# Hello1024/shared-tensor

Measured on AMD Instinct MI355X. Metric: async-DP tokens/sec GPT-2-small, higher is better.
Workload: dtype bf16; 1 GPU; model=gpt2-small, global_batch=64, seq_len=1024, parallelism=async-dp1, codec=1bit, n_params=124439808, paramsync=n/a at n_gpus=1 (no links)

## Files before the change

build.py:

```python
#!/usr/bin/env python3
import argparse
import hashlib
import os
import subprocess
import sysconfig

ROOT = os.path.dirname(os.path.abspath(__file__))
CSRC = os.path.join(ROOT, "sharedtensor_amd", "csrc")
OUT = os.path.join(ROOT, "sharedtensor_amd", "_core.so")
BUILD = os.path.join(ROOT, "build")

SOURCES = [
    "codec_cpu.cpp",
    "engine.cpp",
    "rccl_transport.cpp",
    "hip_kernels.hip",
    "ln_kernels.hip",
    "ce_kernels.hip",
    "gelu_kernels.hip",
    "swiglu_kernels.hip",
    "bindings.cpp",
]

HEADERS = ["common.h", "codec_cpu.h", "engine.h", "hip_api.h", "rccl_transport.h"]


def pybind11_include():
    import pybind11
    return pybind11.get_include()


def build(force=False, debug=False, verbose=True):
    os.makedirs(BUILD, exist_ok=True)
    py_inc = sysconfig.get_paths()["include"]
    rocm = os.environ.get("ROCM_PATH", "/opt/rocm")
    hipcc = os.path.join(rocm, "bin", "hipcc")
    cxxflags = [
        "--offload-arch=gfx950",
        "-std=c++20",
        "-O3" if not debug else "-O0",
        "-g" if debug else "",
        "-fPIC",
        "-DSHAMD_WITH_HIP",
        f"-I{CSRC}",
        f"-I{py_inc}",
        f"-I{pybind11_include()}",
        f"-I{rocm}/include",
        "-Wno-unused-result",
        "-fvisibility=hidden",
        "-DNDEBUG" if not debug else "",
        "-parallel-jobs=4",
    ]
    cxxflags = [f for f in cxxflags if f]

    h = hashlib.sha256()
    for f in SOURCES + HEADERS:
        with open(os.path.join(CSRC, f), "rb") as fh:
            h.update(fh.read())
    h.update(" ".join(cxxflags).encode())
    stamp = os.path.join(BUILD, "core.stamp")
    digest = h.hexdigest()
    if not force and os.path.exists(OUT) and os.path.exists(stamp):
        with open(stamp) as fh:
            if fh.read().strip() == digest:
                if verbose:
                    print(f"[build.py] {OUT} up to date")
                return OUT

    objs = []
    procs = []
    for src in SOURCES:
        obj = os.path.join(BUILD, src.replace("/", "_") + ".o")
        objs.append(obj)
        cmd = [hipcc, "-c", os.path.join(CSRC, src), "-o", obj] + cxxflags
        if verbose:
            print("[build.py]", " ".join(cmd))
        procs.append(subprocess.Popen(cmd))
    rc = 0
    for p in procs:
        rc |= p.wait()
    if rc:
        raise RuntimeError("hipcc compilation failed")

    link = [hipcc, "-shared", "-fPIC", "-o", OUT] + objs + [
        f"-L{rocm}/lib", "-lamdhip64", "-lrccl", "-pthread",
        f"-Wl,-rpath,{rocm}/lib",
    ]
    if verbose:
        print("[build.py]", " ".join(link))
    subprocess.check_call(link)
    nm = subprocess.run(["nm", "-C", "-u", OUT], capture_output=True, text=True)
    bad = [l for l in nm.stdout.splitlines() if "shamd::" in l]
    if bad:
        raise RuntimeError("unresolved engine symbols:\n" + "\n".join(bad))
    with open(stamp, "w") as fh:
        fh.write(digest)
    if verbose:
        print(f"[build.py] built {OUT}")
    return OUT


if __name__ == "__main__":
    ap = argparse.ArgumentParser()
    ap.add_argument("--force", action="store_true")
    ap.add_argument("--debug", action="store_true")
    args = ap.parse_args()
    build(force=args.force, debug=args.debug)
```

sharedtensor_amd/csrc/bindings.cpp:

```cpp
#include <pybind11/pybind11.h>
#include <pybind11/stl.h>

#include "codec_cpu.h"
#include "engine.h"
#include "rccl_transport.h"

namespace py = pybind11;
using namespace shamd;

namespace {

py::tuple py_cpu_encode(int codec, uintptr_t delta, int64_t n, double scale_in,
                        uintptr_t payload_out) {
  Codec c = static_cast<Codec>(codec);
  float* d = reinterpret_cast<float*>(delta);
  float scale = scale_in < 0 ? cpu_compute_scale(c, d, n)
                             : static_cast<float>(scale_in);
  cpu_quantize(c, d, n, scale, reinterpret_cast<uint8_t*>(payload_out));
  return py::make_tuple(scale, payload_bytes(c, n));
}

void py_cpu_apply(int codec, uintptr_t payload, int64_t n, double scale,
                  std::vector<uintptr_t> dsts) {
  std::vector<float*> d;
// ... 138 lines not shown
      .def("copy_to", &Engine::copy_to,
           py::call_guard<py::gil_scoped_release>())
      .def("fused_sgd", &Engine::fused_sgd,
           py::call_guard<py::gil_scoped_release>())
      .def("fused_sgd_bf16", &Engine::fused_sgd_bf16,
           py::call_guard<py::gil_scoped_release>())
      .def("fused_adamw", &Engine::fused_adamw,
           py::call_guard<py::gil_scoped_release>())
      .def("notify_dirty", &Engine::notify_dirty)
      .def("close", &Engine::close, py::call_guard<py::gil_scoped_release>())
      .def("is_master", &Engine::is_master)
      .def("listen_port", &Engine::listen_port)
      .def("last_error", &Engine::last_error)
      .def("reconnect_count", &Engine::reconnect_count)
      .def("recent_scales_sent", &Engine::recent_scales_sent)
      .def("recent_scales_recv", &Engine::recent_scales_recv)
      .def("link_stats", [](Engine& e) {
        py::list out;
        for (auto& s : e.link_stats()) {
          py::dict d;
          d["rounds_sent"] = s.rounds_sent;
          d["rounds_recv"] = s.rounds_recv;
          d["bytes_sent"] = s.bytes_sent;
          d["bytes_recv"] = s.bytes_recv;
          d["last_scale_sent"] = s.last_scale_sent;
          d["last_scale_recv"] = s.last_scale_recv;
          d["active"] = s.active;
          d["dead"] = s.dead;
          d["peer"] = s.peer;
          d["rccl"] = s.rccl;
          out.append(d);
        }
        return out;
      });

  py::class_<DevCodec>(m, "DevCodec")
      .def(py::init<int, std::vector<int64_t>, int, bool>(), py::arg("codec"),
           py::arg("sizes"), py::arg("device"), py::arg("delta_bf16") = false)
      .def("reduce_scales", &DevCodec::reduce_scales)
      .def("quantize", &DevCodec::quantize, py::arg("delta"),
           py::arg("scales"), py::arg("payload"), py::arg("stream"),
           py::arg("stats") = 0)
      .def("finalize_scales", &DevCodec::finalize_scales)
      .def("apply", &DevCodec::apply);
  m.def("gpu_add_scatter", &py_gpu_add_scatter, py::arg("src"), py::arg("n"),
        py::arg("alpha"), py::arg("dsts"), py::arg("stream"),
        py::arg("delta_bf16") = false);
  m.def("gpu_fused_sgd", &py_gpu_fused_sgd, py::arg("mom"), py::arg("grad"),
        py::arg("lr"), py::arg("mu"), py::arg("n"), py::arg("dsts"),
        py::arg("stream"), py::arg("delta_bf16") = false);
  m.def("rccl_loopback_payload", &rccl_loopback_payload,
        "Self ncclSend/ncclRecv of a real payload on one device (1-rank "
        "comm): executes the non-blocking enqueue ordering + stream polling "
        "the 2-GPU xGMI links use and verifies the moved bytes.");
  m.def("rccl_self_test", &rccl_self_test,
        py::call_guard<py::gil_scoped_release>());

  m.def("gelu_fwd", [](uintptr_t x, uintptr_t y, int64_t n, uintptr_t stream) {
    hip_gelu_fwd(reinterpret_cast<const void*>(x), reinterpret_cast<void*>(y),
                 n, reinterpret_cast<hipStream_t>(stream));
  });
  m.def("gelu_bwd", [](uintptr_t dy, uintptr_t x, uintptr_t dx, int64_t n,
                       uintptr_t stream) {
    hip_gelu_bwd(reinterpret_cast<const void*>(dy),
                 reinterpret_cast<const void*>(x),
                 reinterpret_cast<void*>(dx), n,
                 reinterpret_cast<hipStream_t>(stream));
  });

  m.def("ce_fwd", [](uintptr_t logits, uintptr_t targets, uintptr_t loss,
                     uintptr_t row_m, uintptr_t row_lse, int64_t R, int64_t V,
                     uintptr_t stream) {
    hip_ce_fwd(reinterpret_cast<const void*>(logits),
               reinterpret_cast<const int32_t*>(targets),
               reinterpret_cast<float*>(loss), reinterpret_cast<float*>(row_m),
               reinterpret_cast<float*>(row_lse), R, V,
               reinterpret_cast<hipStream_t>(stream));
  });
  m.def("ce_bwd", [](uintptr_t logits, uintptr_t targets, uintptr_t row_lse,
                     uintptr_t dlogits, uintptr_t gscale_dev, double inv_r,
                     int64_t R, int64_t V, uintptr_t stream) {
    hip_ce_bwd(reinterpret_cast<const void*>(logits),
               reinterpret_cast<const int32_t*>(targets),
               reinterpret_cast<const float*>(row_lse),
               reinterpret_cast<void*>(dlogits),
               reinterpret_cast<const float*>(gscale_dev),
               static_cast<float>(inv_r), R, V,
               reinterpret_cast<hipStream_t>(stream));
  });

  m.def("ln_fwd", [](uintptr_t x, uintptr_t w, uintptr_t b, uintptr_t y,
                     uintptr_t mean, uintptr_t rstd, int64_t R, int C,
                     double eps, uintptr_t stream) {
    hip_ln_fwd(reinterpret_cast<const void*>(x),
               reinterpret_cast<const void*>(w),
               reinterpret_cast<const void*>(b), reinterpret_cast<void*>(y),
               reinterpret_cast<float*>(mean), reinterpret_cast<float*>(rstd),
               R, C, static_cast<float>(eps),
               reinterpret_cast<hipStream_t>(stream));
  });
  m.def("colsum_bf16", [](uintptr_t x, uintptr_t out, int64_t R, int C,
                          uintptr_t stream) {
    hip_colsum_bf16(reinterpret_cast<const void*>(x),
                    reinterpret_cast<float*>(out), R, C,
                    reinterpret_cast<hipStream_t>(stream));
  });
  m.def("swiglu_fwd", [](uintptr_t x1, uintptr_t x3, uintptr_t y, int64_t n,
                         uintptr_t stream) {
    hip_swiglu_fwd(reinterpret_cast<const void*>(x1),
                   reinterpret_cast<const void*>(x3),
                   reinterpret_cast<void*>(y), n,
                   reinterpret_cast<hipStream_t>(stream));
  });
  m.def("swiglu_bwd", [](uintptr_t dy, uintptr_t x1, uintptr_t x3,
                         uintptr_t dx1, uintptr_t dx3, int64_t n,
                         uintptr_t stream) {
    hip_swiglu_bwd(reinterpret_cast<const void*>(dy),
                   reinterpret_cast<const void*>(x1),
                   reinterpret_cast<const void*>(x3),
                   reinterpret_cast<void*>(dx1),
                   reinterpret_cast<void*>(dx3), n,
                   reinterpret_cast<hipStream_t>(stream));
  });
  m.def("rms_fwd", [](uintptr_t x, uintptr_t w, uintptr_t y, uintptr_t rstd,
                      int64_t R, int C, double eps, uintptr_t stream) {
    hip_rms_fwd(reinterpret_cast<const void*>(x),
                reinterpret_cast<const void*>(w), reinterpret_cast<void*>(y),
                reinterpret_cast<float*>(rstd), R, C, static_cast<float>(eps),
                reinterpret_cast<hipStream_t>(stream));
  });
  m.def("rms_bwd", [](uintptr_t dy, uintptr_t x, uintptr_t w, uintptr_t rstd,
                      uintptr_t dx, uintptr_t dgamma, int64_t R, int C,
                      uintptr_t stream) {
    hip_rms_bwd(reinterpret_cast<const void*>(dy),
                reinterpret_cast<const void*>(x),
                reinterpret_cast<const void*>(w),
                reinterpret_cast<const float*>(rstd),
                reinterpret_cast<void*>(dx), reinterpret_cast<float*>(dgamma),
                R, C, reinterpret_cast<hipStream_t>(stream));
  });
  m.def("ln_bwd", [](uintptr_t dy, uintptr_t x, uintptr_t w, uintptr_t mean,
                     uintptr_t rstd, uintptr_t dx, uintptr_t dgamma,
                     uintptr_t dbeta, int64_t R, int C, uintptr_t stream) {
    hip_ln_bwd(reinterpret_cast<const void*>(dy),
               reinterpret_cast<const void*>(x),
               reinterpret_cast<const void*>(w),
               reinterpret_cast<const float*>(mean),
               reinterpret_cast<const float*>(rstd),
               reinterpret_cast<void*>(dx), reinterpret_cast<float*>(dgamma),
               reinterpret_cast<float*>(dbeta), R, C,
               reinterpret_cast<hipStream_t>(stream));
  });

  m.def("msg_bytes", &Engine::msg_bytes);
  m.def("scales_area", &Engine::scales_area);
  m.def("payload_bytes",
        [](int c, int64_t n) { return payload_bytes(static_cast<Codec>(c), n); });
  m.def("pad64", &pad64);
  m.def("cpu_encode", &py_cpu_encode);
  m.def("cpu_apply", &py_cpu_apply);
  m.def("cpu_scale", &py_cpu_scale);
  m.def("f32_to_e4m3", [](float x) { return static_cast<int>(f32_to_e4m3(x)); });
  m.def("e4m3_to_f32", [](int v) { return e4m3_to_f32(static_cast<uint8_t>(v)); });

#ifdef SHAMD_WITH_HIP
  m.attr("with_hip") = true;
#else
  m.attr("with_hip") = false;
#endif
}
```

sharedtensor_amd/csrc/codec_cpu.cpp:

```cpp
#include "codec_cpu.h"

#include <atomic>
#include <cmath>
#include <cstdlib>
#include <cstring>
#include <thread>
#include <vector>

namespace shamd {

static constexpr int64_t PF_CHUNK = int64_t(1) << 22;

static int cpu_codec_threads() {
  static const int t = [] {
    const char* e = std::getenv("SHTENS_CPU_THREADS");
    if (e) {
      int v = std::atoi(e);
      return v < 1 ? 1 : v;
    }
    unsigned hw = std::thread::hardware_concurrency();
    return static_cast<int>(hw < 1 ? 1 : (hw > 16 ? 16 : hw));
  }();
  return t;
}

void cpu_pfor(int64_t n, const std::function<void(int64_t, int64_t)>& fn) {
  if (n <= 0) return;
  int64_t nchunks = (n + PF_CHUNK - 1) / PF_CHUNK;
  int nt = cpu_codec_threads();
  if (nchunks == 1 || nt == 1) {
    fn(0, n);
    return;
  }
  if (static_cast<int64_t>(nt) > nchunks) nt = static_cast<int>(nchunks);
  std::atomic<int64_t> next{0};
  auto worker = [&] {
    for (;;) {
      int64_t c = next.fetch_add(1, std::memory_order_relaxed);
      if (c >= nchunks) return;
      int64_t lo = c * PF_CHUNK;
      int64_t hi = lo + PF_CHUNK < n ? lo + PF_CHUNK : n;
      fn(lo, hi);
    }
  };
  std::vector<std::thread> ths;
  ths.reserve(nt - 1);
  for (int i = 1; i < nt; ++i) ths.emplace_back(worker);
  worker();
  for (auto& t : ths) t.join();
}

uint8_t f32_to_e4m3(float xf) {
  if (xf != xf) return 0x7F;
  float cl = xf > 448.f ? 448.f : (xf < -448.f ? -448.f : xf);
  uint32_t u;
  std::memcpy(&u, &cl, 4);
  uint8_t sign = (u >> 24) & 0x80;
  uint32_t abs = u & 0x7FFFFFFFu;
  if (abs == 0) return sign;
  int e = static_cast<int>(abs >> 23) - 127;
  uint32_t mant = (abs & 0x7FFFFFu) | 0x800000u;
  int shift = (e >= -6) ? 20 : (14 - e);
  if (shift > 24) return sign;
  uint32_t q = mant >> shift;
  uint32_t rem = mant & ((1u << shift) - 1);
  uint32_t half = 1u << (shift - 1);
  if (rem > half || (rem == half && (q & 1))) q++;
  if (e >= -6) {
    if (q == 16) { q = 8; e++; }
    return sign | static_cast<uint8_t>(((e + 7) << 3) | (q - 8));
  }
  if (q >= 8) return sign | 0x08;
  return sign | static_cast<uint8_t>(q);
}

float e4m3_to_f32(uint8_t v) {
  int sign = (v & 0x80) ? -1 : 1;
  uint32_t exp = (v >> 3) & 0xF;
  uint32_t man = v & 0x7;
  if (exp == 0xF && man == 0x7) return NAN;
  if (exp == 0) return sign * std::ldexp(static_cast<float>(man), -9);
  return sign * std::ldexp(8.0f + man, static_cast<int>(exp) - 10);
}

float pow2_floor_f(double x) {
  if (!(x > 0.0) || std::isinf(x) || std::isnan(x)) return 0.0f;
  int e;
  std::frexp(x, &e);
  return static_cast<float>(std::ldexp(1.0, e - 1));
}

float pow2_ceil_f(double x) {
  if (!(x > 0.0) || std::isinf(x) || std::isnan(x)) return 0.0f;
  int e;
  double m = std::frexp(x, &e);
  return static_cast<float>(std::ldexp(1.0, m == 0.5 ? e - 1 : e));
}

float cpu_compute_scale(Codec c, const float* delta, int64_t n, int stride) {
  if (n <= 0) return 0.0f;
  if (stride < 1) stride = 1;
  int64_t nchunks = (n + PF_CHUNK - 1) / PF_CHUNK;
  if (c == Codec::OneBit) {
    std::vector<double> part(static_cast<size_t>(nchunks), 0.0);
    std::vector<int64_t> cnts(static_cast<size_t>(nchunks), 0);
    cpu_pfor(n, [&](int64_t lo, int64_t hi) {
      int64_t ci = lo / PF_CHUNK;
      double ss = 0.0;
      int64_t cnt = 0;
      for (int64_t i = lo; i < hi; i += stride, ++cnt) {
        double d = atomic_load_f32(delta + i);
        ss += d * d;
      }
      part[static_cast<size_t>(ci)] = ss;
      cnts[static_cast<size_t>(ci)] = cnt;
    });
    double ss = 0.0;
    int64_t cnt = 0;
    for (int64_t ci = 0; ci < nchunks; ++ci) {
      ss += part[static_cast<size_t>(ci)];
      cnt += cnts[static_cast<size_t>(ci)];
    }
    return pow2_floor_f(std::sqrt(ss / static_cast<double>(cnt)));
  }
  std::vector<float> partm(static_cast<size_t>(nchunks), 0.0f);
  cpu_pfor(n, [&](int64_t lo, int64_t hi) {
    int64_t ci = lo / PF_CHUNK;
    float mx = 0.0f;
    for (int64_t i = lo; i < hi; i += stride) {
      float a = std::fabs(atomic_load_f32(delta + i));
      if (a > mx) mx = a;
    }
    partm[static_cast<size_t>(ci)] = mx;
  });
  float mx = 0.0f;
  for (float m : partm)
    if (m > mx) mx = m;
  if (mx == 0.0f || std::isnan(mx) || std::isinf(mx)) return 0.0f;
  return pow2_ceil_f(mx / (c == Codec::Fp8 ? 448.0 : 7.0));
}

void cpu_quantize(Codec c, float* delta, int64_t n, float scale, uint8_t* payload) {
  int64_t pb = payload_bytes(c, n);
  std::memset(payload, 0, pb);
  if (scale == 0.0f) return;
  switch (c) {
    case Codec::OneBit:
      cpu_pfor(n, [&](int64_t lo, int64_t hi) {
        for (int64_t i = lo; i < hi; ++i) {
          float v = atomic_load_f32(delta + i);
          float sent;
          if (v > 0.0f) {
            sent = scale;
          } else {
            payload[i / 8] |= 1u << (i % 8);
            sent = -scale;
          }
          atomic_add_f32(delta + i, -sent);
        }
      });
      break;
    case Codec::Fp8: {
      float inv = 1.0f / scale;
      cpu_pfor(n, [&](int64_t lo, int64_t hi) {
        for (int64_t i = lo; i < hi; ++i) {
          float v = atomic_load_f32(delta + i);
          float sc = v * inv;
          sc = sc > 448.f ? 448.f : (sc < -448.f ? -448.f : sc);
          uint8_t q = f32_to_e4m3(sc);
          payload[i] = q;
          atomic_add_f32(delta + i, -e4m3_to_f32(q) * scale);
        }
      });
      break;
    }
    case Codec::Int4: {
      float inv = 1.0f / scale;
      cpu_pfor(n, [&](int64_t lo, int64_t hi) {
        for (int64_t i = lo; i < hi; ++i) {
          float v = atomic_load_f32(delta + i);
          float r = std::nearbyintf(v * inv);
          r = r > 7.f ? 7.f : (r < -7.f ? -7.f : r);
          int8_t q = static_cast<int8_t>(r);
          payload[i / 2] |= static_cast<uint8_t>(q & 0xF) << ((i % 2) * 4);
          atomic_add_f32(delta + i, -static_cast<float>(q) * scale);
        }
      });
      break;
    }
  }
}

void cpu_apply(Codec c, const uint8_t* payload, int64_t n, float scale,
               float* const* dsts, int ndst) {
  if (scale == 0.0f) return;
  cpu_pfor(n, [&](int64_t lo, int64_t hi) {
    for (int64_t i = lo; i < hi; ++i) {
      float v = 0.0f;
      switch (c) {
        case Codec::OneBit: {
          int bit = (payload[i / 8] >> (i % 8)) & 1;
          v = bit ? -scale : scale;
          break;
        }
        case Codec::Fp8:
          v = e4m3_to_f32(payload[i]) * scale;
          break;
        case Codec::Int4: {
          int8_t q =
              static_cast<int8_t>((payload[i / 2] >> ((i % 2) * 4)) & 0xF);
          if (q > 7) q -= 16;
          v = static_cast<float>(q) * scale;
          break;
        }
      }
      if (v != 0.0f)
        for (int d = 0; d < ndst; ++d) atomic_add_f32(dsts[d] + i, v);
    }
  });
}

void cpu_add_scatter(const float* src, int64_t n, float* const* dsts, int ndst) {
  cpu_pfor(n, [&](int64_t lo, int64_t hi) {
    for (int64_t i = lo; i < hi; ++i) {
      float v = src[i];
      if (v != 0.0f)
        for (int d = 0; d < ndst; ++d) atomic_add_f32(dsts[d] + i, v);
    }
  });
}

}
```

sharedtensor_amd/csrc/hip_api.h:

```cpp
#pragma once

#include <hip/hip_runtime.h>

#include "common.h"

namespace shamd {

inline int64_t align8(int64_t x) { return (x + 7) & ~int64_t(7); }

struct DevTable {
  int64_t* offs = nullptr;
  int64_t* poffs = nullptr;
  int T = 0;
  int64_t n = 0;
  int64_t pe = 0;
};


void hip_reduce_scales(Codec c, const void* delta, bool delta_bf16,
                       const DevTable& tb, void* reduce_buf, float* scales_out,
                       int sample_stride, hipStream_t s);

void hip_quantize(Codec c, void* delta, bool delta_bf16, const DevTable& tb,
                  const float* scales_dev, uint8_t* payload, hipStream_t s,
                  void* stats_out = nullptr);

void hip_finalize_scales(Codec c, const DevTable& tb, const void* reduce_buf,
                         float* scales_out, int sample_stride, hipStream_t s);

void hip_apply(Codec c, const uint8_t* payload, const DevTable& tb,
               const float* scales_dev, float* values, void* d1, void* d2,
               bool delta_bf16, hipStream_t s);

void hip_add_scatter(const float* src, int64_t n, float alpha, float* values,
                     void* d1, void* d2, void* d3, bool delta_bf16,
                     hipStream_t s);

void hip_snapshot_capture(const float* values, void* delta, bool delta_bf16,
                          float* out, int64_t n, hipStream_t s);

void hip_add_delta_scatter(const void* src_delta, bool delta_bf16, int64_t n,
                           float* values, void* d1, void* d2, hipStream_t s);

void hip_fused_sgd(float* mom, const float* grad, float lr, float momentum,
                   int64_t n, float* values, void* d1, void* d2, void* d3,
                   bool delta_bf16, hipStream_t s);

void hip_fused_sgd_bf16(float* mom, const uint16_t* grad, uint16_t* shadow,
                        float lr, float momentum, int64_t n, float* values,
                        void* d1, void* d2, void* d3, bool delta_bf16,
                        hipStream_t s);

void hip_fused_adamw(float* mom, float* vel, const void* grad, bool grad_bf16,
                     uint16_t* shadow, float lr, float beta1, float beta2,
                     float eps, float wd, float inv_bc1, float inv_bc2,
                     int64_t n, float* values, void* d1, void* d2, void* d3,
                     bool delta_bf16, hipStream_t s);

void hip_ln_fwd(const void* x, const void* w, const void* b, void* y,
                float* mean, float* rstd, int64_t R, int C, float eps,
                hipStream_t s);
void hip_ln_bwd(const void* dy, const void* x, const void* w,
                const float* mean, const float* rstd, void* dx, float* dgamma,
                float* dbeta, int64_t R, int C, hipStream_t s);

void hip_colsum_bf16(const void* x, float* out, int64_t R, int C,
                     hipStream_t s);

void hip_rms_fwd(const void* x, const void* w, void* y, float* rstd,
                 int64_t R, int C, float eps, hipStream_t s);
void hip_rms_bwd(const void* dy, const void* x, const void* w,
                 const float* rstd, void* dx, float* dgamma, int64_t R, int C,
                 hipStream_t s);

void hip_ce_fwd(const void* logits, const int32_t* targets, float* loss,
                float* row_m, float* row_lse, int64_t R, int64_t V,
                hipStream_t s);
void hip_ce_bwd(const void* logits, const int32_t* targets,
                const float* row_lse, void* dlogits, const float* gscale_dev,
                float inv_r, int64_t R, int64_t V, hipStream_t s);

void hip_swiglu_fwd(const void* x1, const void* x3, void* y, int64_t n,
                    hipStream_t s);
void hip_swiglu_bwd(const void* dy, const void* x1, const void* x3, void* dx1,
                    void* dx3, int64_t n, hipStream_t s);

void hip_gelu_fwd(const void* x, void* y, int64_t n, hipStream_t s);
void hip_gelu_bwd(const void* dy, const void* x, void* dx, int64_t n,
                  hipStream_t s);

}
```

sharedtensor_amd/models/gpt2.py:

```python
from __future__ import annotations

import math
from dataclasses import dataclass

import torch
import torch.nn as nn
import torch.nn.functional as F


@dataclass
class GPT2Config:
    vocab_size: int = 50257
    n_layer: int = 12
    n_head: int = 12
    n_embd: int = 768
    block_size: int = 1024
    dropout: float = 0.0

    @classmethod
    def small(cls):
        return cls()

    @classmethod
    def tiny(cls):
        return cls(vocab_size=256, n_layer=2, n_head=2, n_embd=64,
                   block_size=64)


class FusedLayerNorm(nn.LayerNorm):

    def forward(self, x):
        if (x.is_cuda and x.dtype == torch.bfloat16
                and self.weight.dtype == torch.bfloat16):
            from ..ops import fused_ln
            if fused_ln.can_use(x, self.weight):
                return fused_ln.fused_layer_norm(x, self.weight, self.bias,
                                                 self.eps)
            with torch.autocast("cuda", enabled=False):
                return F.layer_norm(x, self.normalized_shape, self.weight,
                                    self.bias, self.eps)
        return super().forward(x)


class CausalSelfAttention(nn.Module):
    def __init__(self, cfg: GPT2Config):
        super().__init__()
        assert cfg.n_embd % cfg.n_head == 0
        self.qkv = nn.Linear(cfg.n_embd, 3 * cfg.n_embd)
        self.proj = nn.Linear(cfg.n_embd, cfg.n_embd)
        self.n_head = cfg.n_head
        self.head_dim = cfg.n_embd // cfg.n_head

    def forward(self, x):
        B, T, C = x.shape
        q, k, v = self.qkv(x).split(C, dim=2)
        q = q.view(B, T, self.n_head, self.head_dim).transpose(1, 2)
        k = k.view(B, T, self.n_head, self.head_dim).transpose(1, 2)
        v = v.view(B, T, self.n_head, self.head_dim).transpose(1, 2)
        if x.is_cuda:
            from torch.nn.attention import SDPBackend, sdpa_kernel
            with sdpa_kernel([SDPBackend.EFFICIENT_ATTENTION,
                              SDPBackend.FLASH_ATTENTION, SDPBackend.MATH],
                             set_priority=True):
                y = F.scaled_dot_product_attention(q, k, v, is_causal=True)
        else:
            y = F.scaled_dot_product_attention(q, k, v, is_causal=True)
        y = y.transpose(1, 2).contiguous().view(B, T, C)
        return self.proj(y)


class MLP(nn.Module):
    def __init__(self, cfg: GPT2Config):
        super().__init__()
        self.fc = nn.Linear(cfg.n_embd, 4 * cfg.n_embd)
        self.proj = nn.Linear(4 * cfg.n_embd, cfg.n_embd)

    def forward(self, x):
        return self.proj(F.gelu(self.fc(x), approximate="tanh"))


class Block(nn.Module):
    def __init__(self, cfg: GPT2Config):
        super().__init__()
        self.ln1 = FusedLayerNorm(cfg.n_embd)
        self.attn = CausalSelfAttention(cfg)
        self.ln2 = FusedLayerNorm(cfg.n_embd)
        self.mlp = MLP(cfg)

    def forward(self, x):
        x = x + self.attn(self.ln1(x))
        x = x + self.mlp(self.ln2(x))
        return x


class GPT2(nn.Module):
    def __init__(self, cfg: GPT2Config):
        super().__init__()
        self.cfg = cfg
        self.wte = nn.Embedding(cfg.vocab_size, cfg.n_embd)
        self.wpe = nn.Embedding(cfg.block_size, cfg.n_embd)
        self.blocks = nn.ModuleList(Block(cfg) for _ in range(cfg.n_layer))
        self.ln_f = FusedLayerNorm(cfg.n_embd)
        self.lm_head = nn.Linear(cfg.n_embd, cfg.vocab_size, bias=False)
        self.lm_head.weight = self.wte.weight
        self.apply(self._init)
        for name, p in self.named_parameters():
            if name.endswith("proj.weight"):
                nn.init.normal_(p, std=0.02 / math.sqrt(2 * cfg.n_layer))

    @staticmethod
    def _init(m):
        if isinstance(m, nn.Linear):
            nn.init.normal_(m.weight, std=0.02)
            if m.bias is not None:
                nn.init.zeros_(m.bias)
        elif isinstance(m, nn.Embedding):
            nn.init.normal_(m.weight, std=0.02)

    def forward(self, idx, targets=None):
        B, T = idx.shape
        pos = torch.arange(T, device=idx.device)
        x = self.wte(idx) + self.wpe(pos)
        for blk in self.blocks:
            x = blk(x)
        x = self.ln_f(x)
        logits = self.lm_head(x)
        if targets is None:
            return logits, None
        flat = logits.view(-1, logits.size(-1))
        tgt = targets.reshape(-1)
        if flat.is_cuda and flat.dtype == torch.bfloat16:
            from ..ops import fused_ce
            if fused_ce.can_use(flat):
                return logits, fused_ce.fused_cross_entropy(flat, tgt)
        loss = F.cross_entropy(flat, tgt)
        return logits, loss

    def num_params(self) -> int:
        return sum(p.numel() for p in self.parameters())
```

sharedtensor_amd/ops/fused_ln.py:

```python
from __future__ import annotations

import torch

from .. import _core

MAX_C = 4096


class _FusedLayerNormFn(torch.autograd.Function):
    @staticmethod
    def forward(ctx, x, weight, bias, eps):
        x = x.contiguous()
        C = x.shape[-1]
        R = x.numel() // C
        y = torch.empty_like(x)
        mean = torch.empty(R, dtype=torch.float32, device=x.device)
        rstd = torch.empty(R, dtype=torch.float32, device=x.device)
        s = torch.cuda.current_stream(x.device).cuda_stream
        _core.ln_fwd(x.data_ptr(), weight.data_ptr(),
                     bias.data_ptr() if bias is not None else 0,
                     y.data_ptr(), mean.data_ptr(), rstd.data_ptr(), R, C,
                     float(eps), s)
        ctx.save_for_backward(x, weight, mean, rstd)
        ctx.has_bias = bias is not None
        return y

    @staticmethod
    def backward(ctx, dy):
        x, w, mean, rstd = ctx.saved_tensors
        dy = dy.contiguous()
        C = x.shape[-1]
        R = x.numel() // C
        dx = torch.empty_like(x)
        dwdb = torch.zeros(2 * C, dtype=torch.float32, device=x.device)
        dgamma, dbeta = dwdb[:C], dwdb[C:]
        s = torch.cuda.current_stream(x.device).cuda_stream
        _core.ln_bwd(dy.data_ptr(), x.data_ptr(), w.data_ptr(),
                     mean.data_ptr(), rstd.data_ptr(), dx.data_ptr(),
                     dgamma.data_ptr(), dbeta.data_ptr(), R, C, s)
        return (dx, dgamma.to(w.dtype),
                dbeta.to(w.dtype) if ctx.has_bias else None, None)


def fused_layer_norm(x: torch.Tensor, weight: torch.Tensor,
                     bias: torch.Tensor, eps: float) -> torch.Tensor:
    return _FusedLayerNormFn.apply(x, weight, bias, eps)


def can_use(x: torch.Tensor, weight: torch.Tensor) -> bool:
    return (x.is_cuda and x.dtype == torch.bfloat16
            and weight.dtype == torch.bfloat16
            and x.shape[-1] == weight.numel() and x.shape[-1] <= MAX_C
            and x.shape[-1] % 2 == 0)
```

Before: 745,500 tokens/s.

## Fuse residual add and projection bias into LayerNorm with wave-per-row kernels

Adds wave-per-row HIP kernels that fold the residual add, and optionally the preceding projection bias, into the LayerNorm forward pass. The backward kernel produces the input gradient including the residual gradient, plus dgamma, dbeta and the bias gradient, using per-block partial sums followed by a separate reduce kernel. GPT-2 blocks are restructured to carry the pending residual delta into the next LayerNorm, which removes separate elementwise add and bias kernels and their extra memory passes. The change adds a cached partial-sum buffer and more complex autograd plumbing, and it shifts bf16 rounding points.

```diff
diff --git a/build.py b/build.py
--- a/build.py
+++ b/build.py
@@ -16,6 +16,7 @@
     "rccl_transport.cpp",
     "hip_kernels.hip",
     "ln_kernels.hip",
+    "add_ln_kernels.hip",
     "ce_kernels.hip",
     "gelu_kernels.hip",
     "swiglu_kernels.hip",
diff --git a/sharedtensor_amd/csrc/add_ln_kernels.hip b/sharedtensor_amd/csrc/add_ln_kernels.hip
--- /dev/null
+++ b/sharedtensor_amd/csrc/add_ln_kernels.hip
@@ -0,0 +1,393 @@
+#include <hip/hip_runtime.h>
+
+#include <stdexcept>
+#include <string>
+
+#include "hip_api.h"
+
+namespace shamd {
+
+#define HIP_CHECK_ALN(expr)                                                \
+  do {                                                                     \
+    hipError_t _e = (expr);                                                \
+    if (_e != hipSuccess)                                                  \
+      throw std::runtime_error(std::string("HIP error: ") +                \
+                               hipGetErrorString(_e));                     \
+  } while (0)
+
+static __device__ __forceinline__ uint32_t aln_f32_to_bf16(float f) {
+  uint32_t u = __float_as_uint(f);
+  if ((u & 0x7FFFFFFFu) > 0x7F800000u) return 0x7FC0u;
+  u += 0x7FFFu + ((u >> 16) & 1u);
+  return u >> 16;
+}
+
+static __device__ __forceinline__ void aln_unpack(uint2 p, float* v) {
+  v[0] = __uint_as_float(p.x << 16);
+  v[1] = __uint_as_float(p.x & 0xFFFF0000u);
+  v[2] = __uint_as_float(p.y << 16);
+  v[3] = __uint_as_float(p.y & 0xFFFF0000u);
+}
+
+static __device__ __forceinline__ uint2 aln_pack(const float* v) {
+  uint2 p;
+  p.x = aln_f32_to_bf16(v[0]) | (aln_f32_to_bf16(v[1]) << 16);
+  p.y = aln_f32_to_bf16(v[2]) | (aln_f32_to_bf16(v[3]) << 16);
+  return p;
+}
+
+static __device__ __forceinline__ float aln_wave_sum(float v) {
+#pragma unroll
+  for (int o = 32; o > 0; o >>= 1) v += __shfl_xor(v, o, 64);
+  return v;
+}
+
+constexpr int ALN_FWD_THREADS = 256;
+constexpr int ALN_BWD_THREADS = 256;
+constexpr int ALN_BWD_WAVES = ALN_BWD_THREADS / 64;
+constexpr int ALN_MAX_BLOCKS = 1024;
+constexpr int ALN_MAX_NV = 4;
+
+template <int NV>
+__global__ __launch_bounds__(ALN_FWD_THREADS) void k_add_ln_fwd(
+    const uint16_t* __restrict__ x, const uint16_t* __restrict__ delta,
+    const uint16_t* __restrict__ dbias, const uint16_t* __restrict__ w,
+    const uint16_t* __restrict__ b, uint16_t* __restrict__ x_new,
+    uint16_t* __restrict__ y, float* __restrict__ mean,
+    float* __restrict__ rstd, int64_t R, float eps) {
+  constexpr int C = NV * 256;
+  const int lane = threadIdx.x & 63;
+  const int64_t r =
+      static_cast<int64_t>(blockIdx.x) * (ALN_FWD_THREADS / 64) +
+      __builtin_amdgcn_readfirstlane(threadIdx.x >> 6);
+  if (r >= R) return;
+  const uint2* xr = reinterpret_cast<const uint2*>(x + r * C);
+  float v[NV][4];
+  uint2 px[NV];
+#pragma unroll
+  for (int k = 0; k < NV; ++k) px[k] = xr[k * 64 + lane];
+  if (delta) {
+    const uint2* dr = reinterpret_cast<const uint2*>(delta + r * C);
+    uint2* xo = reinterpret_cast<uint2*>(x_new + r * C);
+    uint2 pd[NV];
+#pragma unroll
+    for (int k = 0; k < NV; ++k) pd[k] = dr[k * 64 + lane];
+#pragma unroll
+    for (int k = 0; k < NV; ++k) {
+      float a[4], d[4];
+      aln_unpack(px[k], a);
+      aln_unpack(pd[k], d);
+#pragma unroll
+      for (int j = 0; j < 4; ++j) a[j] += d[j];
+      if (dbias) {
+        float bb[4];
+        aln_unpack(reinterpret_cast<const uint2*>(dbias)[k * 64 + lane], bb);
+#pragma unroll
+        for (int j = 0; j < 4; ++j) a[j] += bb[j];
+      }
+      uint2 o = aln_pack(a);
+      xo[k * 64 + lane] = o;
+      aln_unpack(o, v[k]);
+    }
+  } else {
+#pragma unroll
+    for (int k = 0; k < NV; ++k) aln_unpack(px[k], v[k]);
+  }
+  float s = 0.f;
+#pragma unroll
+  for (int k = 0; k < NV; ++k) s += (v[k][0] + v[k][1]) + (v[k][2] + v[k][3]);
+  const float m = aln_wave_sum(s) * (1.f / C);
+  float q = 0.f;
+#pragma unroll
+  for (int k = 0; k < NV; ++k)
+#pragma unroll
+    for (int j = 0; j < 4; ++j) {
+      float d = v[k][j] - m;
+      q += d * d;
+    }
+  const float rs = rsqrtf(aln_wave_sum(q) * (1.f / C) + eps);
+  if (lane == 0) {
+    mean[r] = m;
+    rstd[r] = rs;
+  }
+  uint2* yr = reinterpret_cast<uint2*>(y + r * C);
+#pragma unroll
+  for (int k = 0; k < NV; ++k) {
+    float ww[4], o[4];
+    aln_unpack(reinterpret_cast<const uint2*>(w)[k * 64 + lane], ww);
+#pragma unroll
+    for (int j = 0; j < 4; ++j) o[j] = (v[k][j] - m) * rs * ww[j];
+    if (b) {
+      float bb[4];
+      aln_unpack(reinterpret_cast<const uint2*>(b)[k * 64 + lane], bb);
+#pragma unroll
+      for (int j = 0; j < 4; ++j) o[j] += bb[j];
+    }
+    yr[k * 64 + lane] = aln_pack(o);
+  }
+}
+
+template <int NV, bool DDB>
+__global__ __launch_bounds__(ALN_BWD_THREADS) void k_add_ln_bwd(
+    const uint16_t* __restrict__ dy, const uint16_t* __restrict__ xn,
+    const uint16_t* __restrict__ w, const float* __restrict__ mean,
+    const float* __restrict__ rstd, const uint16_t* __restrict__ dres,
+    uint16_t* __restrict__ dx, float* __restrict__ partial, int64_t R) {
+  constexpr int C = NV * 256;
+  constexpr int NS = DDB ? 3 : 2;
+  __shared__ float4 red[NS * C / 4];
+  const int lane = threadIdx.x & 63;
+  const int wave = __builtin_amdgcn_readfirstlane(threadIdx.x >> 6);
+  float ag[NV][4], ab[NV][4], ad[DDB ? NV : 1][4];
+  uint2 pw[NV];
+#pragma unroll
+  for (int k = 0; k < NV; ++k) {
+    pw[k] = reinterpret_cast<const uint2*>(w)[k * 64 + lane];
+#pragma unroll
+    for (int j = 0; j < 4; ++j) {
+      ag[k][j] = 0.f;
+      ab[k][j] = 0.f;
+      if constexpr (DDB) ad[k][j] = 0.f;
+    }
+  }
+  const int64_t stride = static_cast<int64_t>(gridDim.x) * ALN_BWD_WAVES;
+#pragma unroll 1
+  for (int64_t r = static_cast<int64_t>(blockIdx.x) * ALN_BWD_WAVES + wave;
+       r < R; r += stride) {
+    const uint2* dyr = reinterpret_cast<const uint2*>(dy + r * C);
+    const uint2* xr = reinterpret_cast<const uint2*>(xn + r * C);
+    uint2 pg[NV], px[NV], pr[NV];
+#pragma unroll
+    for (int k = 0; k < NV; ++k) pg[k] = dyr[k * 64 + lane];
+#pragma unroll
+    for (int k = 0; k < NV; ++k) px[k] = xr[k * 64 + lane];
+    if (dres) {
+      const uint2* rr = reinterpret_cast<const uint2*>(dres + r * C);
+#pragma unroll
+      for (int k = 0; k < NV; ++k) pr[k] = rr[k * 64 + lane];
+    }
+    const float m = mean[r], rs = rstd[r];
+    float s1 = 0.f, s2 = 0.f;
+#pragma unroll
+    for (int k = 0; k < NV; ++k) {
+      float d[4], xv[4], ww[4];
+      aln_unpack(pg[k], d);
+      aln_unpack(px[k], xv);
+      aln_unpack(pw[k], ww);
+#pragma unroll
+      for (int j = 0; j < 4; ++j) {
+        const float h = (xv[j] - m) * rs;
+        const float g = d[j] * ww[j];
+        ag[k][j] += d[j] * h;
+        ab[k][j] += d[j];
+        s1 += g;
+        s2 += g * h;
+      }
+    }
+#pragma unroll
+    for (int o = 32; o > 0; o >>= 1) {
+      const float u1 = __shfl_xor(s1, o, 64), u2 = __shfl_xor(s2, o, 64);
+      s1 += u1;
+      s2 += u2;
+    }
+    const float t1 = s1 * (1.f / C), t2 = s2 * (1.f / C);
+    uint2* dxr = reinterpret_cast<uint2*>(dx + r * C);
+#pragma unroll
+    for (int k = 0; k < NV; ++k) {
+      float d[4], xv[4], ww[4], o[4];
+      aln_unpack(pg[k], d);
+      aln_unpack(px[k], xv);
+      aln_unpack(pw[k], ww);
+#pragma unroll
+      for (int j = 0; j < 4; ++j)
+        o[j] = (d[j] * ww[j] - t1 - (xv[j] - m) * rs * t2) * rs;
+      if (dres) {
+        float rv[4];
+        aln_unpack(pr[k], rv);
+#pragma unroll
+        for (int j = 0; j < 4; ++j) o[j] += rv[j];
+      }
+      if constexpr (DDB) {
+#pragma unroll
+        for (int j = 0; j < 4; ++j) ad[k][j] += o[j];
+      }
+      dxr[k * 64 + lane] = aln_pack(o);
+    }
+  }
+#pragma unroll 1
+  for (int wv = 0; wv < ALN_BWD_WAVES; ++wv) {
+    if (wave == wv) {
+#pragma unroll
+      for (int k = 0; k < NV; ++k) {
+        const int i = k * 64 + lane;
+        float4 a = make_float4(ag[k][0], ag[k][1], ag[k][2], ag[k][3]);
+        float4 bsum = make_float4(ab[k][0], ab[k][1], ab[k][2], ab[k][3]);
+        if (wv != 0) {
+          float4 p = red[i], q = red[C / 4 + i];
+          a.x += p.x; a.y += p.y; a.z += p.z; a.w += p.w;
+          bsum.x += q.x; bsum.y += q.y; bsum.z += q.z; bsum.w += q.w;
+        }
+        red[i] = a;
+        red[C / 4 + i] = bsum;
+        if constexpr (DDB) {
+          float4 c = make_float4(ad[k][0], ad[k][1], ad[k][2], ad[k][3]);
+          if (wv != 0) {
+            float4 p = red[2 * (C / 4) + i];
+            c.x += p.x; c.y += p.y; c.z += p.z; c.w += p.w;
+          }
+          red[2 * (C / 4) + i] = c;
+        }
+      }
+    }
+    __syncthreads();
+  }
+  float4* pout = reinterpret_cast<float4*>(partial) +
+                 static_cast<int64_t>(blockIdx.x) * (NS * C / 4);
+  for (int i = threadIdx.x; i < NS * C / 4; i += ALN_BWD_THREADS)
+    pout[i] = red[i];
+}
+
+__global__ __launch_bounds__(256) void k_add_ln_reduce(
+    const float* __restrict__ partial, int G, int nsc, int C,
+    uint16_t* __restrict__ o0, uint16_t* __restrict__ o1,
+    uint16_t* __restrict__ o2) {
+  __shared__ float red[16][17];
+  const int cg = threadIdx.x & 15, rg = threadIdx.x >> 4;
+  const int j = blockIdx.x * 16 + cg;
+  float a = 0.f;
+  if (j < nsc)
+    for (int g = rg; g < G; g += 16)
+      a += partial[static_cast<int64_t>(g) * nsc + j];
+  red[rg][cg] = a;
+  __syncthreads();
+  if (rg == 0 && j < nsc) {
+    float t = 0.f;
+#pragma unroll
+    for (int i = 0; i < 16; ++i) t += red[i][cg];
+    const int s = j / C, c = j - s * C;
+    uint16_t* out = s == 0 ? o0 : (s == 1 ? o1 : o2);
+    if (out) out[c] = static_cast<uint16_t>(aln_f32_to_bf16(t));
+  }
+}
+
+bool hip_add_ln_supported(int C) {
+  return C > 0 && C % 256 == 0 && C / 256 <= ALN_MAX_NV;
+}
+
+int hip_add_ln_max_blocks() { return ALN_MAX_BLOCKS; }
+
+static void aln_check_align(const void* p, const char* what) {
+  if (reinterpret_cast<uintptr_t>(p) & 7u)
+    throw std::runtime_error(std::string("add_ln: ") + what +
+                             " is not 8-byte aligned");
+}
+
+void hip_add_ln_fwd(const void* x, const void* delta, const void* dbias,
+                    const void* w, const void* b, void* x_new, void* y,
+                    float* mean, float* rstd, int64_t R, int C, float eps,
+                    hipStream_t s) {
+  if (!hip_add_ln_supported(C)) throw std::runtime_error("add_ln: bad C");
+  if (delta && !x_new) throw std::runtime_error("add_ln: delta needs x_new");
+  if (dbias && !delta) throw std::runtime_error("add_ln: dbias needs delta");
+  aln_check_align(x, "x");
+  aln_check_align(delta, "delta");
+  aln_check_align(dbias, "delta_bias");
+  aln_check_align(w, "weight");
+  aln_check_align(b, "bias");
+  aln_check_align(x_new, "x_new");
+  aln_check_align(y, "y");
+  if (R <= 0) return;
+  constexpr int rows = ALN_FWD_THREADS / 64;
+  const int64_t blocks = (R + rows - 1) / rows;
+  if (blocks > 0x7FFFFFFF) throw std::runtime_error("add_ln: R too large");
+  auto launch = [&](auto kern) {
+    hipLaunchKernelGGL(kern, dim3(static_cast<uint32_t>(blocks)),
+                       dim3(ALN_FWD_THREADS), 0, s,
+                       static_cast<const uint16_t*>(x),
+                       static_cast<const uint16_t*>(delta),
+                       static_cast<const uint16_t*>(dbias),
+                       static_cast<const uint16_t*>(w),
+                       static_cast<const uint16_t*>(b),
+                       static_cast<uint16_t*>(x_new),
+                       static_cast<uint16_t*>(y), mean, rstd, R, eps);
+  };
+  switch (C / 256) {
+    case 1: launch(k_add_ln_fwd<1>); break;
+    case 2: launch(k_add_ln_fwd<2>); break;
+    case 3: launch(k_add_ln_fwd<3>); break;
+    default: launch(k_add_ln_fwd<4>); break;
+  }
+  HIP_CHECK_ALN(hipGetLastError());
+}
+
+template <typename K>
+static int aln_resident_blocks(K kern, int* cache) {
+  int dev = 0;
+  HIP_CHECK_ALN(hipGetDevice(&dev));
+  if (dev < 0 || dev >= 64) dev = 0;
+  if (cache[dev] == 0) {
+    int per_cu = 0, cus = 0;
+    HIP_CHECK_ALN(hipOccupancyMaxActiveBlocksPerMultiprocessor(
+        &per_cu, kern, ALN_BWD_THREADS, 0));
+    HIP_CHECK_ALN(hipDeviceGetAttribute(
+        &cus, hipDeviceAttributeMultiprocessorCount, dev));
+    int g = per_cu * cus;
+    if (g < 1) g = 1;
+    if (g > ALN_MAX_BLOCKS) g = ALN_MAX_BLOCKS;
+    cache[dev] = g;
+  }
+  return cache[dev];
+}
+
+void hip_add_ln_bwd(const void* dy, const void* x_new, const void* w,
+                    const float* mean, const float* rstd, const void* d_x_new,
+                    void* dx_total, void* dgamma, void* dbeta, void* ddbias,
+                    float* partial, int64_t R, int C, hipStream_t s) {
+  if (!hip_add_ln_supported(C)) throw std::runtime_error("add_ln: bad C");
+  aln_check_align(dy, "dy");
+  aln_check_align(x_new, "x_new");
+  aln_check_align(w, "weight");
+  aln_check_align(d_x_new, "d_x_new");
+  aln_check_align(dx_total, "dx_total");
+  if (reinterpret_cast<uintptr_t>(partial) & 15u)
+    throw std::runtime_error("add_ln: partials are not 16-byte aligned");
+  if (R <= 0) throw std::runtime_error("add_ln: empty input");
+  static int cache[ALN_MAX_NV][2][64];
+  int grid = 0;
+  auto launch = [&](auto kern, int* c) {
+    grid = aln_resident_blocks(kern, c);
+    const int64_t need = (R + ALN_BWD_WAVES - 1) / ALN_BWD_WAVES;
+    if (need < grid) grid = static_cast<int>(need);
+    hipLaunchKernelGGL(kern, dim3(grid), dim3(ALN_BWD_THREADS), 0, s,
+                       static_cast<const uint16_t*>(dy),
+                       static_cast<const uint16_t*>(x_new),
+                       static_cast<const uint16_t*>(w), mean, rstd,
+                       static_cast<const uint16_t*>(d_x_new),
+                       static_cast<uint16_t*>(dx_total), partial, R);
+  };
+  const int nv = C / 256;
+  if (ddbias) {
+    switch (nv) {
+      case 1: launch(k_add_ln_bwd<1, true>, cache[0][1]); break;
+      case 2: launch(k_add_ln_bwd<2, true>, cache[1][1]); break;
+      case 3: launch(k_add_ln_bwd<3, true>, cache[2][1]); break;
+      default: launch(k_add_ln_bwd<4, true>, cache[3][1]); break;
+    }
+  } else {
+    switch (nv) {
+      case 1: launch(k_add_ln_bwd<1, false>, cache[0][0]); break;
+      case 2: launch(k_add_ln_bwd<2, false>, cache[1][0]); break;
+      case 3: launch(k_add_ln_bwd<3, false>, cache[2][0]); break;
+      default: launch(k_add_ln_bwd<4, false>, cache[3][0]); break;
+    }
+  }
+  HIP_CHECK_ALN(hipGetLastError());
+  const int nsc = (ddbias ? 3 : 2) * C;
+  hipLaunchKernelGGL(k_add_ln_reduce, dim3(nsc / 16), dim3(256), 0, s, partial,
+                     grid, nsc, C, static_cast<uint16_t*>(dgamma),
+                     static_cast<uint16_t*>(dbeta),
+                     static_cast<uint16_t*>(ddbias));
+  HIP_CHECK_ALN(hipGetLastError());
+}
+
+}
diff --git a/sharedtensor_amd/csrc/bindings.cpp b/sharedtensor_amd/csrc/bindings.cpp
--- a/sharedtensor_amd/csrc/bindings.cpp
+++ b/sharedtensor_amd/csrc/bindings.cpp
@@ -314,6 +314,42 @@
                reinterpret_cast<hipStream_t>(stream));
   });
 
+  m.def("add_ln_supported", &hip_add_ln_supported);
+  m.def("add_ln_max_blocks", &hip_add_ln_max_blocks);
+  m.def("add_ln_fwd", [](uintptr_t x, uintptr_t delta, uintptr_t dbias,
+                         uintptr_t w, uintptr_t b, uintptr_t x_new,
+                         uintptr_t y, uintptr_t mean, uintptr_t rstd,
+                         int64_t R, int C, double eps, uintptr_t stream) {
+    hip_add_ln_fwd(reinterpret_cast<const void*>(x),
+                   reinterpret_cast<const void*>(delta),
+                   reinterpret_cast<const void*>(dbias),
+                   reinterpret_cast<const void*>(w),
+                   reinterpret_cast<const void*>(b),
+                   reinterpret_cast<void*>(x_new), reinterpret_cast<void*>(y),
+                   reinterpret_cast<float*>(mean),
+                   reinterpret_cast<float*>(rstd), R, C,
+                   static_cast<float>(eps),
+                   reinterpret_cast<hipStream_t>(stream));
+  });
+  m.def("add_ln_bwd", [](uintptr_t dy, uintptr_t x_new, uintptr_t w,
+                         uintptr_t mean, uintptr_t rstd, uintptr_t d_x_new,
+                         uintptr_t dx_total, uintptr_t dgamma, uintptr_t dbeta,
+                         uintptr_t ddbias, uintptr_t partial, int64_t R, int C,
+                         uintptr_t stream) {
+    hip_add_ln_bwd(reinterpret_cast<const void*>(dy),
+                   reinterpret_cast<const void*>(x_new),
+                   reinterpret_cast<const void*>(w),
+                   reinterpret_cast<const float*>(mean),
+                   reinterpret_cast<const float*>(rstd),
+                   reinterpret_cast<const void*>(d_x_new),
+                   reinterpret_cast<void*>(dx_total),
+                   reinterpret_cast<void*>(dgamma),
+                   reinterpret_cast<void*>(dbeta),
+                   reinterpret_cast<void*>(ddbias),
+                   reinterpret_cast<float*>(partial), R, C,
+                   reinterpret_cast<hipStream_t>(stream));
+  });
+
   m.def("msg_bytes", &Engine::msg_bytes);
   m.def("scales_area", &Engine::scales_area);
   m.def("payload_bytes",
diff --git a/sharedtensor_amd/csrc/codec_cpu.cpp b/sharedtensor_amd/csrc/codec_cpu.cpp
--- a/sharedtensor_amd/csrc/codec_cpu.cpp
+++ b/sharedtensor_amd/csrc/codec_cpu.cpp
@@ -162,10 +162,11 @@
       break;
     case Codec::Fp8: {
       float inv = 1.0f / scale;
+      const bool div = !std::isfinite(inv);
       cpu_pfor(n, [&](int64_t lo, int64_t hi) {
         for (int64_t i = lo; i < hi; ++i) {
           float v = atomic_load_f32(delta + i);
-          float sc = v * inv;
+          float sc = div ? v / scale : v * inv;
           sc = sc > 448.f ? 448.f : (sc < -448.f ? -448.f : sc);
           uint8_t q = f32_to_e4m3(sc);
           payload[i] = q;
@@ -176,10 +177,11 @@
     }
     case Codec::Int4: {
       float inv = 1.0f / scale;
+      const bool div = !std::isfinite(inv);
       cpu_pfor(n, [&](int64_t lo, int64_t hi) {
         for (int64_t i = lo; i < hi; ++i) {
           float v = atomic_load_f32(delta + i);
-          float r = std::nearbyintf(v * inv);
+          float r = std::nearbyintf(div ? v / scale : v * inv);
           r = r > 7.f ? 7.f : (r < -7.f ? -7.f : r);
           int8_t q = static_cast<int8_t>(r);
           payload[i / 2] |= static_cast<uint8_t>(q & 0xF) << ((i % 2) * 4);
diff --git a/sharedtensor_amd/csrc/hip_api.h b/sharedtensor_amd/csrc/hip_api.h
--- a/sharedtensor_amd/csrc/hip_api.h
+++ b/sharedtensor_amd/csrc/hip_api.h
@@ -64,6 +64,17 @@
                 const float* mean, const float* rstd, void* dx, float* dgamma,
                 float* dbeta, int64_t R, int C, hipStream_t s);
 
+bool hip_add_ln_supported(int C);
+int hip_add_ln_max_blocks();
+void hip_add_ln_fwd(const void* x, const void* delta, const void* dbias,
+                    const void* w, const void* b, void* x_new, void* y,
+                    float* mean, float* rstd, int64_t R, int C, float eps,
+                    hipStream_t s);
+void hip_add_ln_bwd(const void* dy, const void* x_new, const void* w,
+                    const float* mean, const float* rstd, const void* d_x_new,
+                    void* dx_total, void* dgamma, void* dbeta, void* ddbias,
+                    float* partial, int64_t R, int C, hipStream_t s);
+
 void hip_colsum_bf16(const void* x, float* out, int64_t R, int C,
                      hipStream_t s);
 
diff --git a/sharedtensor_amd/models/gpt2.py b/sharedtensor_amd/models/gpt2.py
--- a/sharedtensor_amd/models/gpt2.py
+++ b/sharedtensor_amd/models/gpt2.py
@@ -27,6 +27,9 @@
                    block_size=64)
 
 
+FUSE_PROJ_BIAS = True
+
+
 class FusedLayerNorm(nn.LayerNorm):
 
     def forward(self, x):
@@ -42,6 +45,27 @@
         return super().forward(x)
 
 
+def _fused_ln_ok(ln: nn.LayerNorm, x: torch.Tensor) -> bool:
+    if (x.is_cuda and x.dtype == torch.bfloat16
+            and ln.weight.dtype == torch.bfloat16):
+        from ..ops import fused_ln
+        return fused_ln.can_use(x, ln.weight)
+    return False
+
+
+def add_ln(ln: nn.LayerNorm, x, delta, delta_bias=None):
+    if delta is None:
+        return x, ln(x)
+    if _fused_ln_ok(ln, x):
+        from ..ops import fused_ln
+        return fused_ln.fused_add_layer_norm(x, delta, ln.weight, ln.bias,
+                                             ln.eps, delta_bias)
+    x = x + delta
+    if delta_bias is not None:
+        x = x + delta_bias
+    return x, ln(x)
+
+
 class CausalSelfAttention(nn.Module):
     def __init__(self, cfg: GPT2Config):
         super().__init__()
@@ -51,7 +75,7 @@
         self.n_head = cfg.n_head
         self.head_dim = cfg.n_embd // cfg.n_head
 
-    def forward(self, x):
+    def forward(self, x, proj_bias=True):
         B, T, C = x.shape
         q, k, v = self.qkv(x).split(C, dim=2)
         q = q.view(B, T, self.n_head, self.head_dim).transpose(1, 2)
@@ -66,6 +90,8 @@
         else:
             y = F.scaled_dot_product_attention(q, k, v, is_causal=True)
         y = y.transpose(1, 2).contiguous().view(B, T, C)
+        if not proj_bias:
+            return F.linear(y, self.proj.weight)
         return self.proj(y)
 
 
@@ -75,8 +101,11 @@
         self.fc = nn.Linear(cfg.n_embd, 4 * cfg.n_embd)
         self.proj = nn.Linear(4 * cfg.n_embd, cfg.n_embd)
 
-    def forward(self, x):
-        return self.proj(F.gelu(self.fc(x), approximate="tanh"))
+    def forward(self, x, proj_bias=True):
+        h = F.gelu(self.fc(x), approximate="tanh")
+        if not proj_bias:
+            return F.linear(h, self.proj.weight)
+        return self.proj(h)
 
 
 class Block(nn.Module):
@@ -87,10 +116,13 @@
         self.ln2 = FusedLayerNorm(cfg.n_embd)
         self.mlp = MLP(cfg)
 
-    def forward(self, x):
-        x = x + self.attn(self.ln1(x))
-        x = x + self.mlp(self.ln2(x))
-        return x
+    def forward(self, x, delta=None, delta_bias=None, fuse_proj_bias=False):
+        x, h = add_ln(self.ln1, x, delta, delta_bias)
+        fuse = fuse_proj_bias and _fused_ln_ok(self.ln2, x)
+        a = self.attn(h, proj_bias=not fuse)
+        x, h = add_ln(self.ln2, x, a, self.attn.proj.bias if fuse else None)
+        m = self.mlp(h, proj_bias=not fuse)
+        return x, m, (self.mlp.proj.bias if fuse else None)
 
 
 class GPT2(nn.Module):
@@ -121,9 +153,11 @@
         B, T = idx.shape
         pos = torch.arange(T, device=idx.device)
         x = self.wte(idx) + self.wpe(pos)
+        delta = delta_bias = None
         for blk in self.blocks:
-            x = blk(x)
-        x = self.ln_f(x)
+            x, delta, delta_bias = blk(x, delta, delta_bias,
+                                       FUSE_PROJ_BIAS)
+        _, x = add_ln(self.ln_f, x, delta, delta_bias)
         logits = self.lm_head(x)
         if targets is None:
             return logits, None
diff --git a/sharedtensor_amd/ops/fused_ln.py b/sharedtensor_amd/ops/fused_ln.py
--- a/sharedtensor_amd/ops/fused_ln.py
+++ b/sharedtensor_amd/ops/fused_ln.py
@@ -6,6 +6,63 @@
 
 MAX_C = 4096
 
+_partials: dict = {}
+
+
+def _wave_path(C: int, *tensors) -> bool:
+    return (_core.add_ln_supported(C)
+            and all(t is None or t.data_ptr() % 8 == 0 for t in tensors))
+
+
+def _ptr(t) -> int:
+    return t.data_ptr() if t is not None else 0
+
+
+def _partials_for(device, C: int, stream: int) -> torch.Tensor:
+    key = (device.index, stream)
+    n = _core.add_ln_max_blocks() * 3 * C
+    buf = _partials.get(key)
+    if buf is None or buf.numel() < n:
+        buf = torch.empty(n, dtype=torch.float32, device=device)
+        _partials[key] = buf
+    return buf
+
+
+def _wave_fwd(x, delta, delta_bias, weight, bias, eps):
+    C = x.shape[-1]
+    R = x.numel() // C
+    x_new = torch.empty_like(x) if delta is not None else None
+    y = torch.empty_like(x)
+    mean = torch.empty(R, dtype=torch.float32, device=x.device)
+    rstd = torch.empty(R, dtype=torch.float32, device=x.device)
+    if R:
+        s = torch.cuda.current_stream(x.device).cuda_stream
+        _core.add_ln_fwd(x.data_ptr(), _ptr(delta), _ptr(delta_bias),
+                         weight.data_ptr(), _ptr(bias), _ptr(x_new),
+                         y.data_ptr(), mean.data_ptr(), rstd.data_ptr(), R, C,
+                         float(eps), s)
+    return x_new, y, mean, rstd
+
+
+def _wave_bwd(dy, x_new, weight, mean, rstd, d_x_new, want_ddbias):
+    C = x_new.shape[-1]
+    R = x_new.numel() // C
+    dx = torch.empty_like(x_new)
+    sums = torch.empty(3 if want_ddbias else 2, C, dtype=torch.bfloat16,
+                       device=x_new.device)
+    if R == 0:
+        sums.zero_()
+    else:
+        stream = torch.cuda.current_stream(x_new.device).cuda_stream
+        part = _partials_for(x_new.device, C, stream)
+        _core.add_ln_bwd(dy.data_ptr(), x_new.data_ptr(), weight.data_ptr(),
+                         mean.data_ptr(), rstd.data_ptr(), _ptr(d_x_new),
+                         dx.data_ptr(), sums[0].data_ptr(),
+                         sums[1].data_ptr(),
+                         sums[2].data_ptr() if want_ddbias else 0,
+                         part.data_ptr(), R, C, stream)
+    return dx, sums[0], sums[1], sums[2] if want_ddbias else None
+
 
 class _FusedLayerNormFn(torch.autograd.Function):
     @staticmethod
@@ -13,6 +70,12 @@
         x = x.contiguous()
         C = x.shape[-1]
         R = x.numel() // C
+        ctx.has_bias = bias is not None
+        ctx.wave = _wave_path(C, x, weight, bias)
+        if ctx.wave:
+            _, y, mean, rstd = _wave_fwd(x, None, None, weight, bias, eps)
+            ctx.save_for_backward(x, weight, mean, rstd)
+            return y
         y = torch.empty_like(x)
         mean = torch.empty(R, dtype=torch.float32, device=x.device)
         rstd = torch.empty(R, dtype=torch.float32, device=x.device)
@@ -22,7 +85,6 @@
                      y.data_ptr(), mean.data_ptr(), rstd.data_ptr(), R, C,
                      float(eps), s)
         ctx.save_for_backward(x, weight, mean, rstd)
-        ctx.has_bias = bias is not None
         return y
 
     @staticmethod
@@ -31,6 +93,10 @@
         dy = dy.contiguous()
         C = x.shape[-1]
         R = x.numel() // C
+        if ctx.wave and dy.data_ptr() % 8 == 0:
+            dx, dgamma, dbeta, _ = _wave_bwd(dy, x, w, mean, rstd, None,
+                                             False)
+            return dx, dgamma, dbeta if ctx.has_bias else None, None
         dx = torch.empty_like(x)
         dwdb = torch.zeros(2 * C, dtype=torch.float32, device=x.device)
         dgamma, dbeta = dwdb[:C], dwdb[C:]
@@ -42,9 +108,67 @@
                 dbeta.to(w.dtype) if ctx.has_bias else None, None)
 
 
+class _FusedAddLayerNormFn(torch.autograd.Function):
+
+    @staticmethod
+    def forward(ctx, x, delta, weight, bias, eps, delta_bias):
+        ctx.set_materialize_grads(False)
+        x_new, y, mean, rstd = _wave_fwd(x, delta, delta_bias, weight, bias,
+                                         eps)
+        ctx.save_for_backward(x_new, weight, mean, rstd)
+        ctx.has_bias = bias is not None
+        ctx.has_delta_bias = delta_bias is not None
+        return x_new, y
+
+    @staticmethod
+    def backward(ctx, d_x_new, dy):
+        x_new, w, mean, rstd = ctx.saved_tensors
+        if d_x_new is not None:
+            d_x_new = d_x_new.contiguous()
+        if dy is None:
+            if d_x_new is None:
+                return None, None, None, None, None, None
+            ddb = None
+            if ctx.has_delta_bias:
+                ddb = d_x_new.reshape(-1, d_x_new.shape[-1]).sum(
+                    0, dtype=torch.float32).to(d_x_new.dtype)
+            return d_x_new, d_x_new, None, None, None, ddb
+        dy = dy.contiguous()
+        if dy.data_ptr() % 8 or (d_x_new is not None
+                                 and d_x_new.data_ptr() % 8):
+            dy = dy.clone()
+            d_x_new = d_x_new.clone() if d_x_new is not None else None
+        dx, dgamma, dbeta, ddb = _wave_bwd(dy, x_new, w, mean, rstd, d_x_new,
+                                           ctx.has_delta_bias)
+        return dx, dx, dgamma, dbeta if ctx.has_bias else None, None, ddb
+
+
 def fused_layer_norm(x: torch.Tensor, weight: torch.Tensor,
                      bias: torch.Tensor, eps: float) -> torch.Tensor:
     return _FusedLayerNormFn.apply(x, weight, bias, eps)
+
+
+def fused_add_layer_norm(x: torch.Tensor, delta: torch.Tensor,
+                         weight: torch.Tensor, bias: torch.Tensor, eps: float,
+                         delta_bias: torch.Tensor = None):
+    if delta is None:
+        if delta_bias is not None:
+            raise ValueError("delta_bias without delta")
+        return x, fused_layer_norm(x, weight, bias, eps)
+    if delta.shape != x.shape:
+        raise ValueError("x and delta differ in shape")
+    x = x.contiguous()
+    delta = delta.contiguous()
+    if delta_bias is not None:
+        delta_bias = delta_bias.contiguous()
+    if _wave_path(x.shape[-1], x, delta, weight, bias, delta_bias):
+        return _FusedAddLayerNormFn.apply(x, delta, weight, bias, eps,
+                                          delta_bias)
+    if delta_bias is None:
+        x_new = x + delta
+    else:
+        x_new = (x.float() + delta.float() + delta_bias.float()).to(x.dtype)
+    return x_new, fused_layer_norm(x_new, weight, bias, eps)
 
 
 def can_use(x: torch.Tensor, weight: torch.Tensor) -> bool:
```

Result: faster. 794,100 tokens/s, median of 6 (+6.5%).
